# liuyuan-pal/Gen6D

Hardware: AMD Instinct MI355X
Metric: query images/sec (detect+select+3x refine), 64 ref views (higher is better)
Workload: dtype f32

## Files before the change

gen6d_amd/csrc/common.hip:

```cpp
#include "g6d_common.h"
#include <string.h>
#include <stdint.h>
#include <stdio.h>
#include <atomic>
#include <mutex>
#include <set>
#include <utility>

static thread_local char g_err[256] = "";

void g6d_set_error(const char* msg) {
  strncpy(g_err, msg, sizeof(g_err) - 1);
  g_err[sizeof(g_err) - 1] = 0;
}

int g6d_check_launch(const char* what) {
  hipError_t e = hipGetLastError();
  if (e == hipSuccess) return G6D_OK;
  snprintf(g_err, sizeof(g_err), "%s: %s", what, hipGetErrorString(e));
  return G6D_ELAUNCH;
}

void g6d_allow_lds(const void* func, int bytes) {
  static std::mutex mu;
  static std::set<std::pair<const void*, int>> done;
  int dev = 0;
  (void)hipGetDevice(&dev);
  std::lock_guard<std::mutex> lock(mu);
  if (done.insert({func, dev}).second) (void)hipFuncSetAttribute(func, hipFuncAttributeMaxDynamicSharedMemorySize, bytes);
}

namespace {
struct KnobDef { const char* name; double def; };
const KnobDef kKnobs[G6D_KNOB_COUNT] = {
    {"conv_patch", 1},
    {"tile_policy", 1},
    {"split_target", 512},
    {"patch_pipe", 1},
    {"corr_slots", 512},
    {"sel_rowq", -1},
    {"conv1_mfma", 1},
    {"w43_split_max", 32}, {"w43_split_gain", 0.85}, {"w43_chunk_us", 2.8},
    {"wino_debug", 0},
    {"conv_wino43", 1},
    {"wino_wide", 1},
    {"wino_split_max", 32}, {"wino_split_gain", 0.85}, {"wino_split_fix", 2.0}, {"wino_split_per", 0.6},
    {"wino16_2w", 1},
    {"conv_wino", 1},
    {"conv_wino16", 1},
    {"wino_min_work", -1},
    {"w43_map", 2},
    {"conv_pm", 1},
    {"gemv_mfma", 1},
    {"c16_ablate", 0},
    {"conv16_halo", 1},
    {"conv_narrow", 1},
};
std::atomic<double> g_knob[G6D_KNOB_COUNT];
void knob_defaults() { for (int i = 0; i < G6D_KNOB_COUNT; ++i) g_knob[i].store(kKnobs[i].def, std::memory_order_relaxed); }
struct KnobInit { KnobInit() { knob_defaults(); } } g_knob_init;
}
double g6d_knob(int id) { return g_knob[id].load(std::memory_order_relaxed); }
extern "C" int g6d_set_knob(const char* name, double value) {
  for (int i = 0; name && i < G6D_KNOB_COUNT; ++i)
    if (!strcmp(name, kKnobs[i].name)) { g_knob[i].store(value, std::memory_order_relaxed); return G6D_OK; }
  g6d_set_error("set_knob: unknown knob"); return G6D_EINVAL;
}
extern "C" double g6d_get_knob(const char* name) {
  for (int i = 0; name && i < G6D_KNOB_COUNT; ++i)
    if (!strcmp(name, kKnobs[i].name)) return g_knob[i].load(std::memory_order_relaxed);
  return -1e300;
}
extern "C" void g6d_reset_knobs(void) { knob_defaults(); }

extern "C" int g6d_abi_version(void) { return 12; }
extern "C" const char* g6d_last_error(void) { return g_err; }
extern "C" int g6d_sizeof_conv_desc(void) { return (int)sizeof(G6dConv); }

__global__ void g6d_marker_kernel(int id) { (void)id; }

extern "C" int g6d_marker(int id, g6d_stream_t stream) {
  hipLaunchKernelGGL(g6d_marker_kernel, dim3(1), dim3(64), 0, reinterpret_cast<hipStream_t>(stream), id);
  return g6d_check_launch("g6d_marker");
}

__global__ void g6d_zero_kernel(uint4* p, size_t n16, unsigned char* tail, int ntail) {
  for (size_t i = blockIdx.x * (size_t)blockDim.x + threadIdx.x; i < n16; i += (size_t)gridDim.x * blockDim.x) p[i] = uint4{0u, 0u, 0u, 0u};
  if (blockIdx.x == 0 && (int)threadIdx.x < ntail) tail[threadIdx.x] = 0;
}
// ... 10 lines not shown
```

gen6d_amd/csrc/detector.hip:

```cpp
#include "g6d_common.h"

namespace {

struct LevelStats { float mu[3], sigma[3]; };

__global__ void assemble_kernel(const float* __restrict__ s0, const float* __restrict__ s1, const float* __restrict__ s2,
                                int hc, int wc, int rfn, LevelStats st, float clip, int hs, int ws, int scale_idx,
                                int nch, float* __restrict__ stacked) {
  const long long total = (long long)hs * ws * rfn;
  const long long i = blockIdx.x * (long long)blockDim.x + threadIdx.x;
  if (i >= total) return;
  s0 += (size_t)blockIdx.y * hc * wc * rfn; s1 += (size_t)blockIdx.y * (hc >> 1) * (wc >> 1) * rfn;
  s2 += (size_t)blockIdx.y * (hc >> 2) * (wc >> 2) * rfn; stacked += (size_t)blockIdx.y * total * nch;
  const int r = (int)(i % rfn); const int pix = (int)(i / rfn);
  const int x = pix % ws, y = pix / ws;
  const float ry = (float)hc / (float)hs, rx = (float)wc / (float)ws;
  float sy = ry * (y + 0.5f) - 0.5f; if (sy < 0.f) sy = 0.f;
  float sx = rx * (x + 0.5f) - 0.5f; if (sx < 0.f) sx = 0.f;
  const int y0 = (int)sy, x0 = (int)sx;
  const int y1 = y0 + (y0 < hc - 1), x1 = x0 + (x0 < wc - 1);
  const float ly = sy - y0, lx = sx - x0, hy = 1.f - ly, hx = 1.f - lx;
  const float* src[3] = {s0, s1, s2};
  float* dst = stacked + ((size_t)pix * rfn + r) * nch + 3 * scale_idx;
#pragma unroll
// ... 25 lines not shown
  if (pl < ppb && pix < P) {
    float in[NCH];
    const float* src = stacked + ((size_t)pix * rfn + r) * NCH;
#pragma unroll
    for (int k = 0; k < NCH; ++k) in[k] = src[k];
    typedef float f2 __attribute__((ext_vector_type(2)));
    static_assert(NCH % 2 == 0, "channel pairs");
    f2 inp[NCH / 2];
#pragma unroll
    for (int k = 0; k < NCH / 2; ++k) inp[k] = f2{in[2 * k], in[2 * k + 1]};
    f2 hp[32];
#pragma unroll
    for (int o = 0; o < 64; ++o) {
      f2 a = {b0[o], 0.f};
#pragma unroll
      for (int k = 0; k < NCH / 2; ++k) a = __builtin_elementwise_fma(inp[k], *reinterpret_cast<const f2*>(w0 + o * NCH + 2 * k), a);
      const float v = fmaxf(a.x + a.y, 0.f);
      if (o & 1) hp[o >> 1].y = v; else hp[o >> 1].x = v;
    }
    for (int o = 0; o < 64; ++o) {
      f2 a = {b1[o], 0.f};
#pragma unroll
      for (int k = 0; k < 32; ++k) a = __builtin_elementwise_fma(hp[k], *reinterpret_cast<const f2*>(w1 + o * 64 + 2 * k), a);
      atomicMax(&smax[pl * 64 + o], enc_f(a.x + a.y));
    }
  }
  __syncthreads();
  for (int i = threadIdx.x; i < ppb * 64; i += 256) {
    const int p2 = blockIdx.x * ppb + i / 64;
    if (p2 < P) out[(size_t)p2 * 64 + (i & 63)] = dec_f(smax[i]);
  }
}

__global__ void __launch_bounds__(256) decode_kernel(const float* __restrict__ scores, int ld_s,
                                                     const float* __restrict__ offset, int ld_o,
                                                     const float* __restrict__ scale, int ld_c, int hs, int ws,
                                                     float pool_ratio, float* __restrict__ result) {
  __shared__ float bv[256];
  __shared__ int bi[256];
  const int n = hs * ws;
  scores += (size_t)blockIdx.x * n * ld_s; offset += (size_t)blockIdx.x * n * ld_o; scale += (size_t)blockIdx.x * n * ld_c;
  result += blockIdx.x * 5;
  float best = -INFINITY; int idx = 0x7fffffff;
  for (int i = threadIdx.x; i < n; i += 256) {
    float v = scores[(size_t)i * ld_s];
    if (v > best || (v == best && i < idx)) { best = v; idx = i; }
  }
  bv[threadIdx.x] = best; bi[threadIdx.x] = idx;
  __syncthreads();
  for (int s = 128; s > 0; s >>= 1) {
    if (threadIdx.x < s) {
      float v = bv[threadIdx.x + s]; int j = bi[threadIdx.x + s];
      if (v > bv[threadIdx.x] || (v == bv[threadIdx.x] && j < bi[threadIdx.x])) { bv[threadIdx.x] = v; bi[threadIdx.x] = j; }
    }
    __syncthreads();
  }
  if (threadIdx.x == 0) {
    const int id = bi[0] == 0x7fffffff ? 0 : bi[0];
    const int x = id % ws, y = id / ws;
    result[0] = ((float)x + offset[(size_t)id * ld_o] + 0.5f) * pool_ratio - 0.5f;
    result[1] = ((float)y + offset[(size_t)id * ld_o + 1] + 0.5f) * pool_ratio - 0.5f;
    result[2] = exp2f(scale[(size_t)id * ld_c]);
    result[3] = (float)x; result[4] = (float)y;
  }
}

// ... 47 lines not shown
      for (int e = 0; e < VEC; ++e) {
        const float hx = 1.f - lx[e];
        v[e] = hy * (hx * t00[p_][e] + lx[e] * t01[p_][e]) + ly * (hx * t10[p_][e] + lx[e] * t11[p_][e]);
      }
      if constexpr (VEC == 4) *reinterpret_cast<f32x4*>(d + p_ * dstride) = f32x4{v[0], v[1], v[2], v[3]};
      else d[p_ * dstride] = v[0];
    }
  }
}
}

#define STREAM(s) reinterpret_cast<hipStream_t>(s)

extern "C" int g6d_detector_assemble(const float* s0, const float* s1, const float* s2, int hc, int wc, int rfn,
                                     const float* mu_sigma, float clip, int hs, int ws, int scale_idx, int nch,
                                     float* stacked, int batch, g6d_stream_t stream) {
  if (!s0 || !s1 || !s2 || !mu_sigma || !stacked || hc <= 0 || wc <= 0 || (hc & 3) || (wc & 3) || rfn <= 0 || hs <= 0 || ws <= 0 ||
      scale_idx < 0 || 3 * scale_idx + 3 > nch || batch < 1 || batch > 65535) {
    g6d_set_error("detector_assemble: bad args (level-0 map must be a multiple of 4, hs and ws positive)"); return G6D_EINVAL;
  }
  LevelStats st;
  for (int l = 0; l < 3; ++l) { st.mu[l] = mu_sigma[2 * l]; st.sigma[l] = mu_sigma[2 * l + 1]; }
  const long long total = (long long)hs * ws * rfn;
  hipLaunchKernelGGL(assemble_kernel, dim3((unsigned)((total + 255) / 256), batch), dim3(256), 0, STREAM(stream), s0, s1, s2, hc,
                     wc, rfn, st, clip, hs, ws, scale_idx, nch, stacked);
  return g6d_check_launch("detector_assemble");
}

extern "C" int g6d_detector_score_mlp_max(const float* stacked, int P, int rfn, int nch, const float* w0, const float* b0,
                                          const float* w1, const float* b1, float* out, g6d_stream_t stream) {
  if (!stacked || !w0 || !b0 || !w1 || !b1 || !out || P <= 0 || rfn <= 0 || rfn > 256 || nch != 12) {
    g6d_set_error("detector_score_mlp_max: bad args (rfn <= 256, nch == 12)"); return G6D_EINVAL;
  }
  const int ppb = 256 / rfn;
  hipLaunchKernelGGL(score_mlp_max_kernel<12>, dim3((P + ppb - 1) / ppb), dim3(256), (size_t)ppb * 64 * sizeof(int),
                     STREAM(stream), stacked, P, rfn, w0, b0, w1, b1, out, ppb);
  return g6d_check_launch("detector_score_mlp_max");
}

extern "C" int g6d_detector_decode(const float* scores, int ld_s, const float* offset, int ld_o, const float* scale,
                                   int ld_c, int hs, int ws, int pool_ratio, float* result, int batch, g6d_stream_t stream) {
  if (!scores || !offset || !scale || !result || hs <= 0 || ws <= 0 || batch < 1) { g6d_set_error("detector_decode: bad args"); return G6D_EINVAL; }
  hipLaunchKernelGGL(decode_kernel, dim3(batch), dim3(256), 0, STREAM(stream), scores, ld_s, offset, ld_o, scale, ld_c, hs, ws,
                     (float)pool_ratio, result);
  return g6d_check_launch("detector_decode");
}

extern "C" int g6d_resize_bilinear_pyramid(const float* src, int planes, int H, int W, int nscale, const int* hs, const int* ws,
                                           float* const* dsts, g6d_stream_t stream) {
  if (!src || !hs || !ws || !dsts || planes <= 0 || H <= 0 || W <= 0 || nscale < 1 || nscale > 4) {
    g6d_set_error("resize_bilinear_pyramid: bad args (1..4 destination sizes)"); return G6D_EINVAL;
  }
  PyrArgs a = {};
  a.src = src; a.planes = planes; a.H = H; a.W = W; a.n = nscale;
  bool vec = true;
  for (int k = 0; k < nscale; ++k)
    if (hs[k] <= 0 || ws[k] <= 0 || !dsts[k]) { g6d_set_error("resize_bilinear_pyramid: bad destination"); return G6D_EINVAL; }
    else vec = vec && (ws[k] & 3) == 0 && g6d_aligned16(dsts[k]);
  long long tot = 0;
  for (int k = 0; k < nscale; ++k) {
    a.h[k] = hs[k]; a.w[k] = ws[k]; a.dst[k] = dsts[k]; a.first[k] = tot;
    tot += (long long)((planes + PYR_PL - 1) / PYR_PL) * hs[k] * (vec ? ws[k] / 4 : ws[k]);
  }
  for (int k = nscale; k < 5; ++k) a.first[k] = tot;
  if (tot >= (1ll << 32)) { g6d_set_error("resize_bilinear_pyramid: more than 2^32 work items"); return G6D_EINVAL; }
  const long long blocks = (tot + 255) / 256;
// ... 6 lines not shown
```

gen6d_amd/csrc/g6d_common.h:

```cpp
#pragma once
#include <hip/hip_runtime.h>
#include <stdint.h>
#include "../../include/gen6d_hip.h"

typedef float f32x4 __attribute__((ext_vector_type(4)));
typedef float f32x2 __attribute__((ext_vector_type(2)));
typedef float f32x16 __attribute__((ext_vector_type(16)));

typedef __bf16 bf16x8 __attribute__((ext_vector_type(8)));
typedef _Float16 f16x8 __attribute__((ext_vector_type(8)));

#define G6D_WAVE 64

template <int MM>
__device__ __forceinline__ f32x16 g6d_mfma_lowp(f32x4 alo, f32x4 ahi, f32x4 blo, f32x4 bhi, f32x16 acc) {
  if constexpr (MM == 1) {
    bf16x8 a, b;
#pragma unroll
    for (int i = 0; i < 4; ++i) { a[i] = (__bf16)alo[i]; a[4 + i] = (__bf16)ahi[i]; b[i] = (__bf16)blo[i]; b[4 + i] = (__bf16)bhi[i]; }
    return __builtin_amdgcn_mfma_f32_32x32x16_bf16(a, b, acc, 0, 0, 0);
  } else {
    f16x8 a, b;
#pragma unroll
    for (int i = 0; i < 4; ++i) { a[i] = (_Float16)alo[i]; a[4 + i] = (_Float16)ahi[i]; b[i] = (_Float16)blo[i]; b[4 + i] = (_Float16)bhi[i]; }
// ... 26 lines not shown
__device__ __forceinline__ int g6d_exp_out(const G6dRange16& r) { return r.exps && r.slot_out >= 0 ? r.exps[r.slot_out] : 0; }
__device__ __forceinline__ unsigned g6d_abs_bits(float v) { return __float_as_uint(v) & 0x7fffffffu; }
__device__ __forceinline__ unsigned g6d_wave_max_u(unsigned m) {
#pragma unroll
  for (int o = 32; o > 0; o >>= 1) m = max(m, (unsigned)__shfl_xor((int)m, o, 64));
  return m;
}
__device__ __forceinline__ void g6d_range_max(unsigned* rec, unsigned m) {
  if (m > __hip_atomic_load(rec, __ATOMIC_RELAXED, __HIP_MEMORY_SCOPE_AGENT)) atomicMax(rec, m);
}
__device__ __forceinline__ void g6d_range_record(const G6dRange16& r, unsigned m) {
  if (!r.rec || r.slot_out < 0) return;
  m = g6d_wave_max_u(m);
  if ((threadIdx.x & 63) == 0) g6d_range_max(r.rec + r.slot_out, m);
}
template <int NW>
__device__ __forceinline__ void g6d_range_record_block(const G6dRange16& r, unsigned m) {
  if (!r.rec || r.slot_out < 0) return;
  __shared__ unsigned red[NW];
  m = g6d_wave_max_u(m);
  if ((threadIdx.x & 63) == 0) red[threadIdx.x >> 6] = m;
  __syncthreads();
  if (threadIdx.x == 0) {
#pragma unroll
    for (int w = 1; w < NW; ++w) m = max(m, red[w]);
    g6d_range_max(r.rec + r.slot_out, m);
  }
}

enum G6dKnob {
  G6D_KNOB_CONV_PATCH, G6D_KNOB_TILE_POLICY, G6D_KNOB_SPLIT_TARGET, G6D_KNOB_PATCH_PIPE, G6D_KNOB_CORR_SLOTS, G6D_KNOB_SEL_ROWQ,
  G6D_KNOB_CONV1_MFMA, G6D_KNOB_W43_SPLIT_MAX, G6D_KNOB_W43_SPLIT_GAIN, G6D_KNOB_W43_CHUNK_US, G6D_KNOB_WINO_DEBUG, G6D_KNOB_CONV_WINO43,
  G6D_KNOB_WINO_WIDE, G6D_KNOB_WINO_SPLIT_MAX, G6D_KNOB_WINO_SPLIT_GAIN, G6D_KNOB_WINO_SPLIT_FIX, G6D_KNOB_WINO_SPLIT_PER, G6D_KNOB_WINO16_2W,
  G6D_KNOB_CONV_WINO, G6D_KNOB_CONV_WINO16, G6D_KNOB_WINO_MIN_WORK, G6D_KNOB_W43_MAP, G6D_KNOB_CONV_PM, G6D_KNOB_GEMV_MFMA, G6D_KNOB_C16_ABLATE, G6D_KNOB_CONV16_HALO, G6D_KNOB_CONV_NARROW, G6D_KNOB_COUNT
};
double g6d_knob(int id);

#define G6D_WS_COUNTER_BYTES G6D_WORKSPACE_COUNTER_BYTES
#define G6D_WS_COUNTERS (G6D_WS_COUNTER_BYTES / 4)
__device__ __forceinline__ void g6d_store_wt(float* p, f32x4 v) {
  asm volatile("global_store_dwordx4 %0, %1, off sc1\n\ts_nop 1" ::"v"(p), "v"(v) : "memory");
}
__device__ __forceinline__ bool g6d_split_arrive(int* counter, int splits, int* flag) {
  asm volatile("s_waitcnt vmcnt(0)" ::: "memory");
  __syncthreads();
  if (threadIdx.x == 0) {
    const int last = __hip_atomic_fetch_add(counter, 1, __ATOMIC_RELAXED, __HIP_MEMORY_SCOPE_AGENT) == splits - 1;
    if (last) {
      __hip_atomic_store(counter, 0, __ATOMIC_RELAXED, __HIP_MEMORY_SCOPE_AGENT);
      __builtin_amdgcn_fence(__ATOMIC_ACQUIRE, "agent");
    }
    *flag = last;
  }
  __syncthreads();
  return *flag != 0;
}

struct G6dFin { float* scale; float* shift; int* counter; const double* stats; double inv_count, eps; int n; };
__device__ __forceinline__ void g6d_finalize_stats(const G6dFin& f, int nblocks, int* flag) {
  asm volatile("s_waitcnt vmcnt(0)" ::: "memory");
  __syncthreads();
  if (threadIdx.x == 0) {
    const int last = __hip_atomic_fetch_add(f.counter, 1, __ATOMIC_RELAXED, __HIP_MEMORY_SCOPE_AGENT) == nblocks - 1;
    if (last) {
      __hip_atomic_store(f.counter, 0, __ATOMIC_RELAXED, __HIP_MEMORY_SCOPE_AGENT);
      __builtin_amdgcn_fence(__ATOMIC_ACQUIRE, "agent");
    }
// ... 25 lines not shown
```

gen6d_amd/csrc/vgg_conv1.hip:

```cpp
#ifndef G6D_CONV1_HOST_EMU
#include "g6d_common.h"
#include <stdlib.h>
#define G6D_HD __host__ __device__ __forceinline__
#else
#include <cmath>
#include <cstddef>
#define G6D_HD inline
#endif

#define C1_PTX 32
#define C1_PTY 2
#define C1_IW (2 * C1_PTX + 2)
#define C1_IH (2 * C1_PTY + 2)
#define C1_IWP (C1_IW + 1)
#define C1_CIN 3
#define C1_COUT 64
#define C1_TAPS 27
#define C1_THREADS (C1_PTX * C1_PTY * (C1_COUT / 16))

struct Conv1Norm { float mean[C1_CIN], std[C1_CIN]; int on; };

struct Conv1Smem {
  float in[C1_CIN][C1_IH][C1_IWP];
  float w[C1_TAPS][C1_COUT];
  float b[C1_COUT];
};

G6D_HD void conv1_stage(Conv1Smem& s, int tid, const float* in, const float* w_oihw, const float* bias, int n, int H, int W,
                        int px0, int py0, const Conv1Norm& nm) {
  const int gx0 = 2 * px0 - 1, gy0 = 2 * py0 - 1;
  for (int i = tid; i < C1_CIN * C1_IH * C1_IW; i += C1_THREADS) {
    const int col = i % C1_IW, r = (i / C1_IW) % C1_IH, c = i / (C1_IW * C1_IH);
    const int gy = gy0 + r, gx = gx0 + col;
    const bool ok = gy >= 0 && gy < H && gx >= 0 && gx < W;
// ... 43 lines not shown
#pragma unroll
      for (int k = 0; k < 16; ++k) {
        const int co = cg * 16 + k;
        float m = fmaxf(fmaxf(acc[0][k], acc[1][k]), fmaxf(acc[2][k], acc[3][k])) + s.b[co];
        m = fmaxf(m, 0.f);
        if (nhwc) out[((size_t)(n * Ho + py) * Wo + px) * C1_COUT + co] = m;
        else out[((size_t)(n * C1_COUT + co) * Ho + py) * Wo + px] = m;
      }
    }
  }
}

#ifndef G6D_CONV1_HOST_EMU

namespace {

__global__ void __launch_bounds__(C1_THREADS) vgg_conv1_pool_kernel(const float* __restrict__ in,
                                                                    const float* __restrict__ w_oihw,
                                                                    const float* __restrict__ bias, int H, int W, int Ho,
                                                                    int Wo, float* __restrict__ out, int nhwc, const Conv1Norm nm) {
  __shared__ Conv1Smem s;
  const int px0 = blockIdx.x * C1_PTX, py0 = blockIdx.y * C1_PTY, n = blockIdx.z;
  conv1_stage(s, threadIdx.x, in, w_oihw, bias, n, H, W, px0, py0, nm);
  __syncthreads();
  conv1_compute(s, threadIdx.x, out, n, Ho, Wo, px0, py0, nhwc != 0);
}


#define M1_PTX 32
#define M1_PTY 8
#define M1_IW (2 * M1_PTX + 2)
#define M1_IH (2 * M1_PTY + 2)
#define M1_IWP 80

template <typename OT, bool PAIR = false>
__global__ void __launch_bounds__(256) vgg_conv1_pool_mfma_kernel(const float* __restrict__ in, const float* __restrict__ w_oihw,
                                                                  const float* __restrict__ bias, int H, int W, int Ho, int Wo,
                                                                  OT* __restrict__ out, const Conv1Norm nm, const G6dRange16 rng) {
  __shared__ float tile[C1_CIN][M1_IH][M1_IWP];
  const int tid = threadIdx.x, lane = tid & 63, wave = tid >> 6;
  const int li = lane & 31, lh = lane >> 5;
  const int px0 = blockIdx.x * M1_PTX, py0 = blockIdx.y * M1_PTY, n = blockIdx.z;
  const int gx0 = 2 * px0 - 1, gy0 = 2 * py0 - 1;
  for (int i = tid; i < C1_CIN * M1_IH * M1_IW; i += 256) {
    const int col = i % M1_IW, r = (i / M1_IW) % M1_IH, c = i / (M1_IW * M1_IH);
    const int gy = gy0 + r, gx = gx0 + col;
    const bool ok = gy >= 0 && gy < H && gx >= 0 && gx < W;
    float v = ok ? in[((size_t)(n * C1_CIN + c) * H + gy) * W + gx] : 0.f;
    if (nm.on && ok) v = (v - nm.mean[c]) / nm.std[c];
    tile[c][r][col] = v;
  }
  float wb[2][14];
  int koff[14];
#pragma unroll
  for (int s = 0; s < 14; ++s) {
    const int k = 2 * s + lh;
    const int kk = k < C1_TAPS ? k : 0;
    const int c = kk / 9, ky = (kk % 9) / 3, kx = kk % 3;
    koff[s] = (c * M1_IH + ky) * M1_IWP + kx;
#pragma unroll
    for (int t = 0; t < 2; ++t) wb[t][s] = k < C1_TAPS ? w_oihw[(li + 32 * t) * C1_TAPS + k] : 0.f;
  }
  const float b0 = bias[li], b1 = bias[li + 32];
  __syncthreads();
  const float* tbase = &tile[0][0][0];
  const int q = li >> 2, p = li & 3;
  const int lane_off = (p >> 1) * M1_IWP + 2 * q + (p & 1);
  const int eo = PAIR ? g6d_exp_out(rng) : 0;
  unsigned amax = 0;
#pragma unroll 1
  for (int g = 0; g < 8; ++g) {
    const int ty = 2 * wave + (g >> 2), gx = g & 3;
    const float* a = tbase + (2 * ty) * M1_IWP + 16 * gx + lane_off;
    f32x16 acc0, acc1;
#pragma unroll
    for (int r = 0; r < 16; ++r) { acc0[r] = 0.f; acc1[r] = 0.f; }
#pragma unroll
    for (int s = 0; s < 14; ++s) {
      const float av = a[koff[s]];
      acc0 = __builtin_amdgcn_mfma_f32_32x32x2f32(av, wb[0][s], acc0, 0, 0, 0);
      acc1 = __builtin_amdgcn_mfma_f32_32x32x2f32(av, wb[1][s], acc1, 0, 0, 0);
    }
    const int py = py0 + ty;
    if (py < Ho) {
#pragma unroll
      for (int j = 0; j < 4; ++j) {
        const int px = px0 + 8 * gx + 2 * j + lh;
        if (px < Wo) {
          const float m0 = fmaxf(fmaxf(acc0[4 * j], acc0[4 * j + 1]), fmaxf(acc0[4 * j + 2], acc0[4 * j + 3])) + b0;
          const float m1 = fmaxf(fmaxf(acc1[4 * j], acc1[4 * j + 1]), fmaxf(acc1[4 * j + 2], acc1[4 * j + 3])) + b1;
          OT* o = out + ((size_t)(n * Ho + py) * Wo + px) * (PAIR ? 2 * C1_COUT : C1_COUT);
          float r0 = fmaxf(m0, 0.f), r1 = fmaxf(m1, 0.f);
          if constexpr (PAIR) {
            amax = max(amax, max(g6d_abs_bits(r0), g6d_abs_bits(r1)));
            r0 = ldexpf(r0, -eo); r1 = ldexpf(r1, -eo);
          }
          o[li] = (OT)r0; o[li + 32] = (OT)r1;
          if constexpr (PAIR) { o[C1_COUT + li] = (OT)(r0 - (float)(OT)r0); o[C1_COUT + li + 32] = (OT)(r1 - (float)(OT)r1); }
        }
      }
    }
  }
  if constexpr (PAIR) g6d_range_record(rng, amax);
}

int conv1_launch(const float* in, int N, int H, int W, const float* w_oihw, const float* bias, int Cin, int Cout, float* out,
                 int nhwc, g6d_stream_t stream, const float* mean = nullptr, const float* stdv = nullptr) {
  if (!in || !w_oihw || !bias || !out || N <= 0 || N > 65535 || H < 2 || W < 2 || Cin != C1_CIN || Cout != C1_COUT ||
      (long long)N * Cout * (H / 2) * (W / 2) >= (1ll << 31)) {
    g6d_set_error("vgg_conv1_pool: bad args (3 -> 64 channels, H, W >= 2)"); return G6D_EINVAL;
  }
  const int Ho = H / 2, Wo = W / 2;
  Conv1Norm nm = {};
  if (mean && stdv) {
    for (int c = 0; c < C1_CIN; ++c) { nm.mean[c] = mean[c]; nm.std[c] = stdv[c]; }
    nm.on = 1;
  }
  const bool use_mfma = g6d_knob(G6D_KNOB_CONV1_MFMA) != 0;
  if (nhwc && use_mfma) {
    hipLaunchKernelGGL(vgg_conv1_pool_mfma_kernel<float>, dim3((Wo + M1_PTX - 1) / M1_PTX, (Ho + M1_PTY - 1) / M1_PTY, N), dim3(256), 0,
                       reinterpret_cast<hipStream_t>(stream), in, w_oihw, bias, H, W, Ho, Wo, out, nm,
                       G6dRange16{});
    return g6d_check_launch("vgg_conv1_pool_mfma");
  }
  hipLaunchKernelGGL(vgg_conv1_pool_kernel, dim3((Wo + C1_PTX - 1) / C1_PTX, (Ho + C1_PTY - 1) / C1_PTY, N), dim3(C1_THREADS),
                     0, reinterpret_cast<hipStream_t>(stream), in, w_oihw, bias, H, W, Ho, Wo, out, nhwc, nm);
  return g6d_check_launch("vgg_conv1_pool");
}

}

extern "C" int g6d_vgg_conv1_pool(const float* in, int N, int H, int W, const float* w_oihw, const float* bias, int Cin,
                                  int Cout, float* out, g6d_stream_t stream) {
  return conv1_launch(in, N, H, W, w_oihw, bias, Cin, Cout, out, 0, stream);
}

extern "C" int g6d_vgg_conv1_pool_nhwc(const float* in, int N, int H, int W, const float* w_oihw, const float* bias, int Cin,
                                       int Cout, float* out, g6d_stream_t stream) {
  return conv1_launch(in, N, H, W, w_oihw, bias, Cin, Cout, out, 1, stream);
}

extern "C" int g6d_vgg_conv1_pool_nhwc_norm(const float* in, int N, int H, int W, const float* w_oihw, const float* bias, int Cin,
                                            int Cout, const float* mean_host, const float* std_host, float* out, g6d_stream_t stream) {
  if (!mean_host || !std_host) { g6d_set_error("vgg_conv1_pool_nhwc_norm: mean / std missing"); return G6D_EINVAL; }
  return conv1_launch(in, N, H, W, w_oihw, bias, Cin, Cout, out, 1, stream, mean_host, std_host);
}

extern "C" int g6d_vgg_conv1_pool_nhwc16_ex(const float* in, int N, int H, int W, const float* w_oihw, const float* bias, int Cin, int Cout,
                                            const float* mean_host, const float* std_host, void* out16, int math_mode, const G6dRange16* range,
                                            g6d_stream_t stream) {
  if (!in || !w_oihw || !bias || !out16 || N <= 0 || N > 65535 || H < 2 || W < 2 || Cin != C1_CIN || Cout != C1_COUT ||
      math_mode < 1 || math_mode > 3 || (long long)N * Cout * (H / 2) * (W / 2) >= (1ll << 30)) {
    g6d_set_error("vgg_conv1_pool_nhwc16: bad args (3 -> 64 channels, H, W >= 2, math_mode 1 / 2 / 3)"); return G6D_EINVAL;
  }
  const int Ho = H / 2, Wo = W / 2;
  Conv1Norm nm = {};
  if (mean_host && std_host) {
    for (int c = 0; c < C1_CIN; ++c) { nm.mean[c] = mean_host[c]; nm.std[c] = std_host[c]; }
    nm.on = 1;
  }
  const dim3 grid((Wo + M1_PTX - 1) / M1_PTX, (Ho + M1_PTY - 1) / M1_PTY, N);
  const G6dRange16 rng = range ? *range : G6dRange16{};
  if (math_mode == 1)
    hipLaunchKernelGGL(vgg_conv1_pool_mfma_kernel<__bf16>, grid, dim3(256), 0, reinterpret_cast<hipStream_t>(stream), in, w_oihw, bias, H, W, Ho, Wo,
                       static_cast<__bf16*>(out16), nm, rng);
  else if (math_mode == 2)
    hipLaunchKernelGGL(vgg_conv1_pool_mfma_kernel<_Float16>, grid, dim3(256), 0, reinterpret_cast<hipStream_t>(stream), in, w_oihw, bias, H, W, Ho, Wo,
                       static_cast<_Float16*>(out16), nm, rng);
  else
    hipLaunchKernelGGL((vgg_conv1_pool_mfma_kernel<_Float16, true>), grid, dim3(256), 0, reinterpret_cast<hipStream_t>(stream), in, w_oihw, bias, H, W,
                       Ho, Wo, static_cast<_Float16*>(out16), nm, rng);
  return g6d_check_launch("vgg_conv1_pool_mfma16");
}

extern "C" int g6d_vgg_conv1_pool_nhwc16(const float* in, int N, int H, int W, const float* w_oihw, const float* bias, int Cin, int Cout,
                                         const float* mean_host, const float* std_host, void* out16, int math_mode, g6d_stream_t stream) {
  return g6d_vgg_conv1_pool_nhwc16_ex(in, N, H, W, w_oihw, bias, Cin, Cout, mean_host, std_host, out16, math_mode, nullptr, stream);
}

#else

extern "C" int g6d_conv1_emulate(const float* in, int N, int H, int W, const float* w_oihw, const float* bias, float* out,
                                 int nhwc, const float* mean, const float* stdv) {
  const int Ho = H / 2, Wo = W / 2;
  Conv1Smem* s = new Conv1Smem;
  Conv1Norm nm = {};
  if (mean && stdv) { for (int c = 0; c < C1_CIN; ++c) { nm.mean[c] = mean[c]; nm.std[c] = stdv[c]; } nm.on = 1; }
  for (int n = 0; n < N; ++n)
    for (int by = 0; by < (Ho + C1_PTY - 1) / C1_PTY; ++by)
      for (int bx = 0; bx < (Wo + C1_PTX - 1) / C1_PTX; ++bx) {
        for (int tid = 0; tid < C1_THREADS; ++tid) conv1_stage(*s, tid, in, w_oihw, bias, n, H, W, bx * C1_PTX, by * C1_PTY, nm);
        for (int tid = 0; tid < C1_THREADS; ++tid) conv1_compute(*s, tid, out, n, Ho, Wo, bx * C1_PTX, by * C1_PTY, nhwc != 0);
      }
  delete s;
  return 0;
}

#endif
```

Baseline: 359.6.

## Run detector score MLP with max-pooling on MFMA matrix cores

Adds a wave-per-pixel kernel that evaluates the two-layer score MLP (12→64→64) over all reference views with 32x32x2 f32 MFMA instructions instead of scalar FMAs. Weights are held in registers, the next input row is prefetched, and the max over views is done with ds_swizzle folds instead of LDS atomicMax. The new path is enabled by default when the view count is a multiple of 32 and the input is 8-byte aligned, with a knob to fall back. The trade-off is higher register pressure and a different fp32 accumulation order.

Result: no change. 362.4, median of 6 (+0.8%).

```diff
diff --git a/gen6d_amd/csrc/common.hip b/gen6d_amd/csrc/common.hip
--- a/gen6d_amd/csrc/common.hip
+++ b/gen6d_amd/csrc/common.hip
@@ -55,6 +55,7 @@
     {"c16_ablate", 0},
     {"conv16_halo", 1},
     {"conv_narrow", 1},
+    {"mlp_mfma", 1},
 };
 std::atomic<double> g_knob[G6D_KNOB_COUNT];
 void knob_defaults() { for (int i = 0; i < G6D_KNOB_COUNT; ++i) g_knob[i].store(kKnobs[i].def, std::memory_order_relaxed); }
diff --git a/gen6d_amd/csrc/detector.hip b/gen6d_amd/csrc/detector.hip
--- a/gen6d_amd/csrc/detector.hip
+++ b/gen6d_amd/csrc/detector.hip
@@ -81,6 +81,84 @@
   }
 }
 
+template <int N>
+__device__ __forceinline__ void mlp_fold(float (&v)[32], int col) {
+  const bool up = (col & N) != 0;
+#pragma unroll
+  for (int i = 0; i < N; ++i) {
+    const float keep = up ? v[i + N] : v[i], send = up ? v[i] : v[i + N];
+    const float got = __int_as_float(__builtin_amdgcn_ds_swizzle(__float_as_int(send), (N << 10) | 0x1f));
+    v[i] = fmaxf(keep, got);
+  }
+}
+
+__global__ void __launch_bounds__(256) score_mlp_max_mfma_kernel(const float* __restrict__ stacked, int P, int nt,
+                                                                 const float* __restrict__ w0, const float* __restrict__ b0,
+                                                                 const float* __restrict__ w1, const float* __restrict__ b1,
+                                                                 float* __restrict__ out) {
+  typedef float f2 __attribute__((ext_vector_type(2)));
+  const int lane = threadIdx.x & 63, col = lane & 31, h = lane >> 5;
+  const int wave = blockIdx.x * 4 + (threadIdx.x >> 6), nwave = gridDim.x * 4;
+  if (wave >= P) return;
+  float a0[2][6], a1[2][2][16], bias0[2][16];
+#pragma unroll
+  for (int m = 0; m < 2; ++m) {
+#pragma unroll
+    for (int s = 0; s < 6; ++s) a0[m][s] = w0[(32 * m + col) * 12 + s + 6 * h];
+#pragma unroll
+    for (int r = 0; r < 16; ++r) {
+      const int u = 8 * (r >> 2) + (r & 3) + 4 * h;
+      bias0[m][r] = b0[32 * m + u];
+#pragma unroll
+      for (int mo = 0; mo < 2; ++mo) a1[mo][m][r] = w1[(32 * mo + col) * 64 + 32 * m + u];
+    }
+  }
+  const int oc = 32 * (col >> 4) + 8 * ((col & 15) >> 2) + 4 * h + (col & 3);
+  const float bias1 = b1[oc];
+  auto row = [&](int pix, int j) { return reinterpret_cast<const f2*>(stacked + (((size_t)pix * nt + j) * 32 + col) * 12 + 6 * h); };
+  const f2* src = row(wave, 0);
+  f2 x[3] = {src[0], src[1], src[2]};
+  for (int pix = wave; pix < P; pix += nwave) {
+    float best = -INFINITY;
+    for (int j = 0; j < nt; ++j) {
+      const bool more = j + 1 < nt || pix + nwave < P;
+      const f2* nsrc = !more ? src : (j + 1 < nt ? row(pix, j + 1) : row(pix + nwave, 0));
+      const f2 xn[3] = {nsrc[0], nsrc[1], nsrc[2]};
+      src = nsrc;
+      f32x16 hid[2];
+#pragma unroll
+      for (int m = 0; m < 2; ++m)
+#pragma unroll
+        for (int r = 0; r < 16; ++r) hid[m][r] = bias0[m][r];
+#pragma unroll
+      for (int s = 0; s < 6; ++s)
+#pragma unroll
+        for (int m = 0; m < 2; ++m) hid[m] = __builtin_amdgcn_mfma_f32_32x32x2f32(a0[m][s], x[s >> 1][s & 1], hid[m], 0, 0, 0);
+      f32x16 o[2];
+#pragma unroll
+      for (int mo = 0; mo < 2; ++mo)
+#pragma unroll
+        for (int r = 0; r < 16; ++r) o[mo][r] = 0.f;
+#pragma unroll
+      for (int m = 0; m < 2; ++m)
+#pragma unroll
+        for (int r = 0; r < 16; ++r) {
+          const float hv = fmaxf(hid[m][r], 0.f);
+#pragma unroll
+          for (int mo = 0; mo < 2; ++mo) o[mo] = __builtin_amdgcn_mfma_f32_32x32x2f32(a1[mo][m][r], hv, o[mo], 0, 0, 0);
+        }
+      float v[32];
+#pragma unroll
+      for (int f = 0; f < 32; ++f) v[f] = o[f >> 4][f & 15];
+      mlp_fold<16>(v, col); mlp_fold<8>(v, col); mlp_fold<4>(v, col); mlp_fold<2>(v, col); mlp_fold<1>(v, col);
+      best = fmaxf(best, v[0]);
+#pragma unroll
+      for (int k = 0; k < 3; ++k) x[k] = xn[k];
+    }
+    out[(size_t)pix * 64 + oc] = best + bias1;
+  }
+}
+
 __global__ void __launch_bounds__(256) decode_kernel(const float* __restrict__ scores, int ld_s,
                                                      const float* __restrict__ offset, int ld_o,
                                                      const float* __restrict__ scale, int ld_c, int hs, int ws,
@@ -194,6 +272,11 @@
   if (!stacked || !w0 || !b0 || !w1 || !b1 || !out || P <= 0 || rfn <= 0 || rfn > 256 || nch != 12) {
     g6d_set_error("detector_score_mlp_max: bad args (rfn <= 256, nch == 12)"); return G6D_EINVAL;
   }
+  if (rfn % 32 == 0 && (reinterpret_cast<uintptr_t>(stacked) & 7) == 0 && g6d_knob(G6D_KNOB_MLP_MFMA) != 0) {
+    const int blocks = (P + 3) / 4 < 1024 ? (P + 3) / 4 : 1024;
+    hipLaunchKernelGGL(score_mlp_max_mfma_kernel, dim3(blocks), dim3(256), 0, STREAM(stream), stacked, P, rfn / 32, w0, b0, w1, b1, out);
+    return g6d_check_launch("detector_score_mlp_max");
+  }
   const int ppb = 256 / rfn;
   hipLaunchKernelGGL(score_mlp_max_kernel<12>, dim3((P + ppb - 1) / ppb), dim3(256), (size_t)ppb * 64 * sizeof(int),
                      STREAM(stream), stacked, P, rfn, w0, b0, w1, b1, out, ppb);
diff --git a/gen6d_amd/csrc/g6d_common.h b/gen6d_amd/csrc/g6d_common.h
--- a/gen6d_amd/csrc/g6d_common.h
+++ b/gen6d_amd/csrc/g6d_common.h
@@ -82,7 +82,8 @@
   G6D_KNOB_CONV_PATCH, G6D_KNOB_TILE_POLICY, G6D_KNOB_SPLIT_TARGET, G6D_KNOB_PATCH_PIPE, G6D_KNOB_CORR_SLOTS, G6D_KNOB_SEL_ROWQ,
   G6D_KNOB_CONV1_MFMA, G6D_KNOB_W43_SPLIT_MAX, G6D_KNOB_W43_SPLIT_GAIN, G6D_KNOB_W43_CHUNK_US, G6D_KNOB_WINO_DEBUG, G6D_KNOB_CONV_WINO43,
   G6D_KNOB_WINO_WIDE, G6D_KNOB_WINO_SPLIT_MAX, G6D_KNOB_WINO_SPLIT_GAIN, G6D_KNOB_WINO_SPLIT_FIX, G6D_KNOB_WINO_SPLIT_PER, G6D_KNOB_WINO16_2W,
-  G6D_KNOB_CONV_WINO, G6D_KNOB_CONV_WINO16, G6D_KNOB_WINO_MIN_WORK, G6D_KNOB_W43_MAP, G6D_KNOB_CONV_PM, G6D_KNOB_GEMV_MFMA, G6D_KNOB_C16_ABLATE, G6D_KNOB_CONV16_HALO, G6D_KNOB_CONV_NARROW, G6D_KNOB_COUNT
+  G6D_KNOB_CONV_WINO, G6D_KNOB_CONV_WINO16, G6D_KNOB_WINO_MIN_WORK, G6D_KNOB_W43_MAP, G6D_KNOB_CONV_PM, G6D_KNOB_GEMV_MFMA, G6D_KNOB_C16_ABLATE, G6D_KNOB_CONV16_HALO, G6D_KNOB_CONV_NARROW,
+  G6D_KNOB_MLP_MFMA, G6D_KNOB_COUNT
 };
 double g6d_knob(int id);
 
```

## Add split-f16 MFMA conv1 body and vectorize conv1 input tile staging

Applied to the files above, without the earlier changes.

Adds a second conv1+pool MFMA body that splits inputs and weights into f16 hi/lo pairs with per-block and per-channel exponent scaling. It then runs four 32x32x16 f16 MFMAs per step instead of many 32x32x2 f32 MFMAs, and does the 2x2 pool with DPP quad max. Input tile staging is rewritten to use 16-byte vector global loads and LDS stores, with a halo offset. The default knob value 2 selects the original f32 MFMA compute with only the new staging. The split-f16 body is opt-in and could change accuracy in edge ranges.

New measurement: 364.5 before, 366.3 after, median of 6. Within noise of the previous version (+0.5%).

```diff
diff --git a/gen6d_amd/csrc/common.hip b/gen6d_amd/csrc/common.hip
--- a/gen6d_amd/csrc/common.hip
+++ b/gen6d_amd/csrc/common.hip
@@ -39,7 +39,7 @@
     {"patch_pipe", 1},
     {"corr_slots", 512},
     {"sel_rowq", -1},
-    {"conv1_mfma", 1},
+    {"conv1_mfma", 2},
     {"w43_split_max", 32}, {"w43_split_gain", 0.85}, {"w43_chunk_us", 2.8},
     {"wino_debug", 0},
     {"conv_wino43", 1},
diff --git a/gen6d_amd/csrc/vgg_conv1.hip b/gen6d_amd/csrc/vgg_conv1.hip
--- a/gen6d_amd/csrc/vgg_conv1.hip
+++ b/gen6d_amd/csrc/vgg_conv1.hip
@@ -1,5 +1,6 @@
 #ifndef G6D_CONV1_HOST_EMU
 #include "g6d_common.h"
+#include "pair16.h"
 #include <stdlib.h>
 #define G6D_HD __host__ __device__ __forceinline__
 #else
@@ -109,76 +110,267 @@
 #define M1_IW (2 * M1_PTX + 2)
 #define M1_IH (2 * M1_PTY + 2)
 #define M1_IWP 80
-
-template <typename OT, bool PAIR = false>
+#define M1_TOFF 3
+#define M1_ROWS (C1_CIN * M1_IH)
+#define M1_RLANES 14
+
+typedef unsigned u32x4 __attribute__((ext_vector_type(4)));
+
+__device__ __forceinline__ float c1_quad_max(float v) {
+  float a, b;
+  asm("s_nop 1\n\tv_max_f32_dpp %0, %1, %1 quad_perm:[1,0,3,2] row_mask:0xf bank_mask:0xf bound_ctrl:1" : "=v"(a) : "v"(v));
+  asm("s_nop 1\n\tv_max_f32_dpp %0, %1, %1 quad_perm:[2,3,0,1] row_mask:0xf bank_mask:0xf bound_ctrl:1" : "=v"(b) : "v"(a));
+  return b;
+}
+__device__ __forceinline__ unsigned c1_pack_pair(float u) {
+  const _Float16 hi = (_Float16)u, lo = (_Float16)(u - (float)hi);
+  return (unsigned)__builtin_bit_cast(unsigned short, hi) | ((unsigned)__builtin_bit_cast(unsigned short, lo) << 16);
+}
+__device__ __forceinline__ int c1_exponent(unsigned m) { return max((int)(m >> 23), 1) - 127; }
+
+template <typename OT, bool PAIR, int BODY>
 __global__ void __launch_bounds__(256) vgg_conv1_pool_mfma_kernel(const float* __restrict__ in, const float* __restrict__ w_oihw,
                                                                   const float* __restrict__ bias, int H, int W, int Ho, int Wo,
                                                                   OT* __restrict__ out, const Conv1Norm nm, const G6dRange16 rng) {
-  __shared__ float tile[C1_CIN][M1_IH][M1_IWP];
+  __shared__ __attribute__((aligned(16))) unsigned tile[M1_ROWS * M1_IWP];
+  __shared__ unsigned red[4];
+  __shared__ int wexp[C1_COUT];
   const int tid = threadIdx.x, lane = tid & 63, wave = tid >> 6;
   const int li = lane & 31, lh = lane >> 5;
   const int px0 = blockIdx.x * M1_PTX, py0 = blockIdx.y * M1_PTY, n = blockIdx.z;
   const int gx0 = 2 * px0 - 1, gy0 = 2 * py0 - 1;
-  for (int i = tid; i < C1_CIN * M1_IH * M1_IW; i += 256) {
-    const int col = i % M1_IW, r = (i / M1_IW) % M1_IH, c = i / (M1_IW * M1_IH);
-    const int gy = gy0 + r, gx = gx0 + col;
-    const bool ok = gy >= 0 && gy < H && gx >= 0 && gx < W;
-    float v = ok ? in[((size_t)(n * C1_CIN + c) * H + gy) * W + gx] : 0.f;
-    if (nm.on && ok) v = (v - nm.mean[c]) / nm.std[c];
-    tile[c][r][col] = v;
-  }
-  float wb[2][14];
-  int koff[14];
-#pragma unroll
-  for (int s = 0; s < 14; ++s) {
-    const int k = 2 * s + lh;
-    const int kk = k < C1_TAPS ? k : 0;
-    const int c = kk / 9, ky = (kk % 9) / 3, kx = kk % 3;
-    koff[s] = (c * M1_IH + ky) * M1_IWP + kx;
-#pragma unroll
-    for (int t = 0; t < 2; ++t) wb[t][s] = k < C1_TAPS ? w_oihw[(li + 32 * t) * C1_TAPS + k] : 0.f;
-  }
-  const float b0 = bias[li], b1 = bias[li + 32];
-  __syncthreads();
-  const float* tbase = &tile[0][0][0];
+
+  const int rl = tid / 18, ci = tid - 18 * rl;
+  const bool vec_ok = (W & 3) == 0 && (reinterpret_cast<uintptr_t>(in) & 15u) == 0;
+  float sv[4][4];
+  unsigned tmax = 0;
+#pragma unroll
+  for (int it = 0; it < 4; ++it) {
+    const int row = rl + M1_RLANES * it;
+    const int c = row / M1_IH, r = row - c * M1_IH, gy = gy0 + r;
+    unsigned live = 0;
+#pragma unroll
+    for (int e = 0; e < 4; ++e) sv[it][e] = 0.f;
+    if (rl < M1_RLANES && row < M1_ROWS && gy >= 0 && gy < H) {
+      const float* src = in + ((size_t)(n * C1_CIN + c) * H + gy) * W;
+      if (ci < 16) {
+        const int gx = gx0 + 1 + 4 * ci;
+        if (vec_ok && gx + 3 < W) {
+          const f32x4 t = *reinterpret_cast<const f32x4*>(src + gx);
+#pragma unroll
+          for (int e = 0; e < 4; ++e) sv[it][e] = t[e];
+          live = 15u;
+        } else {
+#pragma unroll
+          for (int e = 0; e < 4; ++e)
+            if (gx + e < W) { sv[it][e] = src[gx + e]; live |= 1u << e; }
+        }
+      } else {
+        const int gx = ci == 16 ? gx0 : gx0 + M1_IW - 1;
+        if (gx >= 0 && gx < W) { sv[it][0] = src[gx]; live = 1u; }
+      }
+    }
+    if (nm.on) {
+      const float mean = c == 0 ? nm.mean[0] : c == 1 ? nm.mean[1] : nm.mean[2];
+      const float sd = c == 0 ? nm.std[0] : c == 1 ? nm.std[1] : nm.std[2];
+#pragma unroll
+      for (int e = 0; e < 4; ++e)
+        if (live >> e & 1u) sv[it][e] = (sv[it][e] - mean) / sd;
+    }
+#pragma unroll
+    for (int e = 0; e < 4; ++e) tmax = max(tmax, g6d_abs_bits(sv[it][e]));
+  }
+  auto put = [&](auto scale) {
+#pragma unroll
+    for (int it = 0; it < 4; ++it) {
+      const int row = rl + M1_RLANES * it;
+      if (rl < M1_RLANES && row < M1_ROWS) {
+        unsigned* t = tile + row * M1_IWP + M1_TOFF;
+        if (ci < 16) {
+          u32x4 q;
+#pragma unroll
+          for (int e = 0; e < 4; ++e) q[e] = scale(sv[it][e]);
+          *reinterpret_cast<u32x4*>(t + 1 + 4 * ci) = q;
+        } else {
+          t[ci == 16 ? 0 : M1_IW - 1] = scale(sv[it][0]);
+        }
+      }
+    }
+  };
   const int q = li >> 2, p = li & 3;
-  const int lane_off = (p >> 1) * M1_IWP + 2 * q + (p & 1);
+  const int lane_off = M1_TOFF + (p >> 1) * M1_IWP + 2 * q + (p & 1);
   const int eo = PAIR ? g6d_exp_out(rng) : 0;
   unsigned amax = 0;
+
+  if constexpr (BODY == 2) {
+    put([](float v) { return __float_as_uint(v); });
+    float wb[2][14];
+    int koff[14];
+#pragma unroll
+    for (int s = 0; s < 14; ++s) {
+      const int k = 2 * s + lh;
+      const int kk = k < C1_TAPS ? k : 0;
+      const int c = kk / 9, ky = (kk % 9) / 3, kx = kk % 3;
+      koff[s] = (c * M1_IH + ky) * M1_IWP + kx;
+#pragma unroll
+      for (int t = 0; t < 2; ++t) wb[t][s] = k < C1_TAPS ? w_oihw[(li + 32 * t) * C1_TAPS + k] : 0.f;
+    }
+    const float b0 = bias[li], b1 = bias[li + 32];
+    __syncthreads();
+    const float* tbase = reinterpret_cast<const float*>(tile);
 #pragma unroll 1
-  for (int g = 0; g < 8; ++g) {
-    const int ty = 2 * wave + (g >> 2), gx = g & 3;
-    const float* a = tbase + (2 * ty) * M1_IWP + 16 * gx + lane_off;
-    f32x16 acc0, acc1;
-#pragma unroll
-    for (int r = 0; r < 16; ++r) { acc0[r] = 0.f; acc1[r] = 0.f; }
-#pragma unroll
-    for (int s = 0; s < 14; ++s) {
-      const float av = a[koff[s]];
-      acc0 = __builtin_amdgcn_mfma_f32_32x32x2f32(av, wb[0][s], acc0, 0, 0, 0);
-      acc1 = __builtin_amdgcn_mfma_f32_32x32x2f32(av, wb[1][s], acc1, 0, 0, 0);
-    }
-    const int py = py0 + ty;
-    if (py < Ho) {
-#pragma unroll
-      for (int j = 0; j < 4; ++j) {
-        const int px = px0 + 8 * gx + 2 * j + lh;
-        if (px < Wo) {
-          const float m0 = fmaxf(fmaxf(acc0[4 * j], acc0[4 * j + 1]), fmaxf(acc0[4 * j + 2], acc0[4 * j + 3])) + b0;
-          const float m1 = fmaxf(fmaxf(acc1[4 * j], acc1[4 * j + 1]), fmaxf(acc1[4 * j + 2], acc1[4 * j + 3])) + b1;
-          OT* o = out + ((size_t)(n * Ho + py) * Wo + px) * (PAIR ? 2 * C1_COUT : C1_COUT);
-          float r0 = fmaxf(m0, 0.f), r1 = fmaxf(m1, 0.f);
-          if constexpr (PAIR) {
-            amax = max(amax, max(g6d_abs_bits(r0), g6d_abs_bits(r1)));
-            r0 = ldexpf(r0, -eo); r1 = ldexpf(r1, -eo);
+    for (int g = 0; g < 8; ++g) {
+      const int ty = 2 * wave + (g >> 2), gx = g & 3;
+      const float* a = tbase + (2 * ty) * M1_IWP + 16 * gx + lane_off;
+      f32x16 acc0, acc1;
+#pragma unroll
+      for (int r = 0; r < 16; ++r) { acc0[r] = 0.f; acc1[r] = 0.f; }
+#pragma unroll
+      for (int s = 0; s < 14; ++s) {
+        const float av = a[koff[s]];
+        acc0 = __builtin_amdgcn_mfma_f32_32x32x2f32(av, wb[0][s], acc0, 0, 0, 0);
+        acc1 = __builtin_amdgcn_mfma_f32_32x32x2f32(av, wb[1][s], acc1, 0, 0, 0);
+      }
+      const int py = py0 + ty;
+      if (py < Ho) {
+#pragma unroll
+        for (int j = 0; j < 4; ++j) {
+          const int px = px0 + 8 * gx + 2 * j + lh;
+          if (px < Wo) {
+            const float m0 = fmaxf(fmaxf(acc0[4 * j], acc0[4 * j + 1]), fmaxf(acc0[4 * j + 2], acc0[4 * j + 3])) + b0;
+            const float m1 = fmaxf(fmaxf(acc1[4 * j], acc1[4 * j + 1]), fmaxf(acc1[4 * j + 2], acc1[4 * j + 3])) + b1;
+            OT* o = out + ((size_t)(n * Ho + py) * Wo + px) * (PAIR ? 2 * C1_COUT : C1_COUT);
+            float r0 = fmaxf(m0, 0.f), r1 = fmaxf(m1, 0.f);
+            if constexpr (PAIR) {
+              amax = max(amax, max(g6d_abs_bits(r0), g6d_abs_bits(r1)));
+              r0 = ldexpf(r0, -eo); r1 = ldexpf(r1, -eo);
+            }
+            o[li] = (OT)r0; o[li + 32] = (OT)r1;
+            if constexpr (PAIR) { o[C1_COUT + li] = (OT)(r0 - (float)(OT)r0); o[C1_COUT + li + 32] = (OT)(r1 - (float)(OT)r1); }
           }
-          o[li] = (OT)r0; o[li + 32] = (OT)r1;
-          if constexpr (PAIR) { o[C1_COUT + li] = (OT)(r0 - (float)(OT)r0); o[C1_COUT + li + 32] = (OT)(r1 - (float)(OT)r1); }
+        }
+      }
+    }
+  } else {
+    tmax = g6d_wave_max_u(tmax);
+    if (lane == 0) red[wave] = tmax;
+    const int arow_ch = 16 * (li >> 3) + 8 * ((li >> 2) & 1) + (li & 3);
+    f16x8 ahi[2][2], alo[2][2];
+#pragma unroll
+    for (int t = 0; t < 2; ++t) {
+      const float* wr = w_oihw + (arow_ch + 4 * t) * C1_TAPS;
+      float wv[2][8];
+      unsigned wm = 0;
+#pragma unroll
+      for (int s = 0; s < 2; ++s)
+#pragma unroll
+        for (int e = 0; e < 8; ++e) {
+          const int k = 16 * s + 8 * lh + e;
+          wv[s][e] = k < C1_TAPS ? wr[k] : 0.f;
+          wm = max(wm, g6d_abs_bits(wv[s][e]));
+        }
+      wm = max(wm, (unsigned)__shfl_xor((int)wm, 32, 64));
+      const int ew = wm != 0 && wm < 0x7f800000u ? c1_exponent(wm) - 8 : 0;
+#pragma unroll
+      for (int s = 0; s < 2; ++s)
+#pragma unroll
+        for (int e = 0; e < 8; ++e) {
+          const float u = ldexpf(wv[s][e], -ew);
+          const _Float16 h = (_Float16)u;
+          ahi[t][s][e] = h; alo[t][s][e] = (_Float16)(u - (float)h);
+        }
+      if (wave == 0 && lh == 0) wexp[arow_ch + 4 * t] = ew;
+    }
+    int koff[2][8];
+#pragma unroll
+    for (int s = 0; s < 2; ++s)
+#pragma unroll
+      for (int e = 0; e < 8; ++e) {
+        const int k = 16 * s + 8 * lh + e;
+        const int kk = k < C1_TAPS ? k : 0;
+        const int c = kk / 9, ky = (kk % 9) / 3, kx = kk % 3;
+        koff[s][e] = (c * M1_IH + ky) * M1_IWP + kx;
+      }
+    const int och = 16 * p + 8 * lh;
+    float b8[8];
+#pragma unroll
+    for (int e = 0; e < 8; ++e) b8[e] = bias[och + e];
+    __syncthreads();
+    tmax = max(max(red[0], red[1]), max(red[2], red[3]));
+    const bool finite = tmax < 0x7f800000u;
+    const int et = finite && tmax != 0 && (tmax < 0x3d800000u || tmax >= 0x46800000u) ? c1_exponent(tmax) : 0;
+    put([et](float v) { return c1_pack_pair(ldexpf(v, -et)); });
+    if (PAIR && !finite) amax = tmax;
+    __syncthreads();
+    int e8[8];
+#pragma unroll
+    for (int e = 0; e < 8; ++e) e8[e] = wexp[och + e] + et;
+#pragma unroll 1
+    for (int g = 0; g < 8; ++g) {
+      const int ty = 2 * wave + (g >> 2), gx = g & 3;
+      const unsigned* a = tile + (2 * ty) * M1_IWP + 16 * gx + lane_off;
+      f32x16 acc[2];
+#pragma unroll
+      for (int t = 0; t < 2; ++t)
+#pragma unroll
+        for (int r = 0; r < 16; ++r) acc[t][r] = 0.f;
+#pragma unroll
+      for (int s = 0; s < 2; ++s) {
+        unsigned x[8];
+#pragma unroll
+        for (int e = 0; e < 8; ++e) x[e] = a[koff[s][e]];
+        u32x4 h4, l4;
+#pragma unroll
+        for (int e = 0; e < 4; ++e) {
+          h4[e] = __builtin_amdgcn_perm(x[2 * e + 1], x[2 * e], 0x05040100u);
+          l4[e] = __builtin_amdgcn_perm(x[2 * e + 1], x[2 * e], 0x07060302u);
+        }
+        const f16x8 bhi = __builtin_bit_cast(f16x8, h4), blo = __builtin_bit_cast(f16x8, l4);
+#pragma unroll
+        for (int t = 0; t < 2; ++t) {
+          acc[t] = __builtin_amdgcn_mfma_f32_32x32x16_f16(alo[t][s], blo, acc[t], 0, 0, 0);
+          acc[t] = __builtin_amdgcn_mfma_f32_32x32x16_f16(alo[t][s], bhi, acc[t], 0, 0, 0);
+          acc[t] = __builtin_amdgcn_mfma_f32_32x32x16_f16(ahi[t][s], blo, acc[t], 0, 0, 0);
+          acc[t] = __builtin_amdgcn_mfma_f32_32x32x16_f16(ahi[t][s], bhi, acc[t], 0, 0, 0);
+        }
+      }
+      float v[8];
+      const bool hi1 = (p & 1) != 0, hi2 = (p & 2) != 0;
+#pragma unroll
+      for (int t = 0; t < 2; ++t)
+#pragma unroll
+        for (int i = 0; i < 4; ++i) {
+          const float m0 = c1_quad_max(acc[t][i]), m1 = c1_quad_max(acc[t][4 + i]);
+          const float m2 = c1_quad_max(acc[t][8 + i]), m3 = c1_quad_max(acc[t][12 + i]);
+          v[4 * t + i] = hi2 ? (hi1 ? m3 : m2) : (hi1 ? m1 : m0);
+        }
+      const int py = py0 + ty, px = px0 + 8 * gx + q;
+      if (py < Ho && px < Wo) {
+#pragma unroll
+        for (int e = 0; e < 8; ++e) v[e] = fmaxf(ldexpf(v[e], e8[e]) + b8[e], 0.f);
+        const size_t pix = (size_t)(n * Ho + py) * Wo + px;
+        if constexpr (PAIR) {
+          c16_store8<3>(v, eo, amax, reinterpret_cast<char*>(out + pix * (2 * C1_COUT) + och), C1_COUT * sizeof(OT));
+        } else if constexpr (sizeof(OT) == 2) {
+          c16_store8<__is_same(OT, __bf16) ? 1 : 2>(v, 0, amax, reinterpret_cast<char*>(out + pix * C1_COUT + och), 0);
+        } else {
+          f32x4* o = reinterpret_cast<f32x4*>(out + pix * C1_COUT + och);
+          o[0] = f32x4{v[0], v[1], v[2], v[3]};
+          o[1] = f32x4{v[4], v[5], v[6], v[7]};
         }
       }
     }
   }
   if constexpr (PAIR) g6d_range_record(rng, amax);
+}
+
+template <typename OT, bool PAIR>
+void conv1_mfma_launch(dim3 grid, hipStream_t stream, const float* in, const float* w_oihw, const float* bias, int H, int W, int Ho, int Wo,
+                       OT* out, const Conv1Norm& nm, const G6dRange16& rng) {
+  if (g6d_knob(G6D_KNOB_CONV1_MFMA) == 2)
+    hipLaunchKernelGGL((vgg_conv1_pool_mfma_kernel<OT, PAIR, 2>), grid, dim3(256), 0, stream, in, w_oihw, bias, H, W, Ho, Wo, out, nm, rng);
+  else
+    hipLaunchKernelGGL((vgg_conv1_pool_mfma_kernel<OT, PAIR, 1>), grid, dim3(256), 0, stream, in, w_oihw, bias, H, W, Ho, Wo, out, nm, rng);
 }
 
 int conv1_launch(const float* in, int N, int H, int W, const float* w_oihw, const float* bias, int Cin, int Cout, float* out,
@@ -195,9 +387,8 @@
   }
   const bool use_mfma = g6d_knob(G6D_KNOB_CONV1_MFMA) != 0;
   if (nhwc && use_mfma) {
-    hipLaunchKernelGGL(vgg_conv1_pool_mfma_kernel<float>, dim3((Wo + M1_PTX - 1) / M1_PTX, (Ho + M1_PTY - 1) / M1_PTY, N), dim3(256), 0,
-                       reinterpret_cast<hipStream_t>(stream), in, w_oihw, bias, H, W, Ho, Wo, out, nm,
-                       G6dRange16{});
+    conv1_mfma_launch<float, false>(dim3((Wo + M1_PTX - 1) / M1_PTX, (Ho + M1_PTY - 1) / M1_PTY, N), reinterpret_cast<hipStream_t>(stream), in,
+                                    w_oihw, bias, H, W, Ho, Wo, out, nm, G6dRange16{});
     return g6d_check_launch("vgg_conv1_pool_mfma");
   }
   hipLaunchKernelGGL(vgg_conv1_pool_kernel, dim3((Wo + C1_PTX - 1) / C1_PTX, (Ho + C1_PTY - 1) / C1_PTY, N), dim3(C1_THREADS),
@@ -238,15 +429,13 @@
   }
   const dim3 grid((Wo + M1_PTX - 1) / M1_PTX, (Ho + M1_PTY - 1) / M1_PTY, N);
   const G6dRange16 rng = range ? *range : G6dRange16{};
+  const hipStream_t st = reinterpret_cast<hipStream_t>(stream);
   if (math_mode == 1)
-    hipLaunchKernelGGL(vgg_conv1_pool_mfma_kernel<__bf16>, grid, dim3(256), 0, reinterpret_cast<hipStream_t>(stream), in, w_oihw, bias, H, W, Ho, Wo,
-                       static_cast<__bf16*>(out16), nm, rng);
+    conv1_mfma_launch<__bf16, false>(grid, st, in, w_oihw, bias, H, W, Ho, Wo, static_cast<__bf16*>(out16), nm, rng);
   else if (math_mode == 2)
-    hipLaunchKernelGGL(vgg_conv1_pool_mfma_kernel<_Float16>, grid, dim3(256), 0, reinterpret_cast<hipStream_t>(stream), in, w_oihw, bias, H, W, Ho, Wo,
-                       static_cast<_Float16*>(out16), nm, rng);
+    conv1_mfma_launch<_Float16, false>(grid, st, in, w_oihw, bias, H, W, Ho, Wo, static_cast<_Float16*>(out16), nm, rng);
   else
-    hipLaunchKernelGGL((vgg_conv1_pool_mfma_kernel<_Float16, true>), grid, dim3(256), 0, reinterpret_cast<hipStream_t>(stream), in, w_oihw, bias, H, W,
-                       Ho, Wo, static_cast<_Float16*>(out16), nm, rng);
+    conv1_mfma_launch<_Float16, true>(grid, st, in, w_oihw, bias, H, W, Ho, Wo, static_cast<_Float16*>(out16), nm, rng);
   return g6d_check_launch("vgg_conv1_pool_mfma16");
 }
 
```
